# brucefan1983/GPUMD

Measured on AMD Instinct MI355X. Metric: atom-steps/sec, NEP PbTe NVE (nep4 2 Te Pb, examples/nep_train/nep.txt), higher is better.
Workload: dtype f32

## Files before the change

### gpumd_amd/csrc/capi_impl.h

```cpp
#pragma once
#include "../../include/nepmi.h"
#include "engine_impl.h"

#include <exception>
#include <string>

struct nepmi_api;
#if defined(NEPMI_CAPI_DISPATCH)
extern "C" const nepmi_api nepmi_self_api;
#define NEPMI_SELF_API (&nepmi_self_api)
#else
#define NEPMI_SELF_API nullptr
#endif

struct nepmi_model {
  const nepmi_api* api;
  nepmi::NepModel m;
};

struct nepmi_engine {
  const nepmi_api* api;
  nepmi::EngineT<NepmiBackend>* e;
};

// ... 584 lines not shown
  e->e->set_unwrapped(d_unwrapped);
  return NEPMI_OK;
}

int nepmi_engine_set_option(nepmi_engine* e, const char* name, double value)
{
  if (!e || !name)
    return fail(NEPMI_ERR_ARG, "null engine or option name");
  const std::string n(name);
  const int iv = (int)value;
  auto& eng = *e->e;
  if (n == "generic")
    return guarded([&] { eng.set_force_generic(iv != 0); });
  if (n == "tiles")
    eng.set_tile_mode(iv < 0 ? -1 : iv > 2 ? 2 : iv);
  else if (n == "win_lanes")
    eng.set_win_lanes(iv);
  else if (n == "win_max_atoms")
    eng.set_win_max_atoms(iv);
  else if (n == "scatter_guard")
    eng.set_scatter_guard_delayed(value, eng.take_guard_delay());
  else if (n == "scatter_guard_hard")
    eng.set_scatter_guard(-1.0, value);
  else if (n == "scatter_guard_delay")
    eng.set_guard_delay(iv);
  else if (n == "radial_mask")
    eng.set_radial_mask(iv != 0);
  else if (n == "radial_sync")
    eng.set_radial_sync(iv != 0);
  else if (n == "angular_fused")
    eng.set_angular_fused(iv != 0);
  else if (n == "angular_pair_trip")
    eng.set_angular_pair_trip(iv != 0);
  else if (n == "fold_seam")
    eng.set_fold_seam(iv != 0);
  else if (n == "brick_force") {
    if (iv != 0 && !eng.has_brick_force())
      return fail(NEPMI_ERR_ARG, "option 'brick_force': the per-brick force kernel is not part of this build (make BRICK=1)");
    eng.set_brick_force(iv != 0);
  }
  else if (n == "win_static")
    eng.set_win2(iv != 0);
  else if (n == "keep_lists_on_box_change")
    eng.set_keep_lists(iv != 0);
  else if (n == "stepwise_loops")
    eng.set_stepwise_loops(iv != 0);
  else if (n == "mfma")
    eng.set_use_mfma(iv);
  else if (n == "angular_recompute")
    eng.set_angular_recompute(iv);
  else
    return fail(NEPMI_ERR_ARG, "unknown engine option '" + n + "'");
  return NEPMI_OK;
}

}
```

### gpumd_amd/csrc/engine.hip

```cpp
#include <hip/hip_runtime.h>
#include <hiprand/hiprand_kernel.h>

#include <cstring>
#include <stdexcept>
#include <string>

#include "engine_impl.h"
#include "nep_scatter.h"
#include "nep_fused.h"
#ifndef NEPMI_WITH_BRICK
#define NEPMI_WITH_BRICK 0
#endif
#if NEPMI_WITH_BRICK
#include "experimental/nep_brick.h"
#endif

namespace nepmi {

#define NEPMI_HIP_CHECK(expr)                                                                       \
  do {                                                                                              \
    hipError_t err__ = (expr);                                                                      \
    if (err__ != hipSuccess)                                                                        \
      throw std::runtime_error(std::string("HIP error: ") + hipGetErrorString(err__) + " at " +     \
                               __FILE__ + ":" + std::to_string(__LINE__) + " (" #expr ")");         \
// ... 1386 lines not shown
    if (t)
      timer_start(timing->slot[slot]);
    hipLaunchKernelGGL((nepmi_kernel_lds_parts<BLOCK, P, Body>), dim3((unsigned)grid), dim3(BLOCK), lds_bytes, stream, body, n,
                       frozen);
    NEPMI_HIP_CHECK(hipGetLastError());
    if (t)
      timer_stop(timing->slot[slot]);
  }

  template <int BLOCK, class Body, bool SORTED = false>
  void launch_lds_pairs(int slot, int64_t n, const Body& body)
  {
    if (n <= 0)
      return;
    const int64_t grid = ((2 * n + BLOCK - 1) / BLOCK + 7) / 8 * 8;
    const size_t lds_bytes = ((size_t)body.lds_floats() * sizeof(float) + 15) / 16 * 16;
    void (*kern)(const Body, const int64_t, const int*) = nullptr;
    if constexpr (SORTED)
      kern = &nepmi_kernel_lds_pairs_sorted<BLOCK, Body>;
    else
      kern = &nepmi_kernel_lds_pairs<BLOCK, Body>;
    if (lds_bytes > 60 * 1024)
      NEPMI_HIP_CHECK(hipFuncSetAttribute(reinterpret_cast<const void*>(kern), hipFuncAttributeMaxDynamicSharedMemorySize, (int)lds_bytes));
    const bool t = timed(slot);
    if (t)
      timer_start(timing->slot[slot]);
    hipLaunchKernelGGL(kern, dim3((unsigned)grid), dim3(BLOCK), lds_bytes, stream, body, n, frozen);
    NEPMI_HIP_CHECK(hipGetLastError());
    if (t)
      timer_stop(timing->slot[slot]);
  }

  template <class S>
  size_t fused_image_floats(const ModelD& md) const
  {
    return (size_t)fused_lds_layout<S>(md).total;
  }
  template <class S>
  void launch_angular_fused(int slot, int64_t n, const ModelD& md, const Bufs& b, int export_qfp, float* img, bool build, bool pair_trip)
  {
    AngularFusedBody<S> body{md, b, export_qfp, nullptr};
    if (build) {
      hipLaunchKernelGGL((nepmi_fused_image<AngularFusedBody<S>>), dim3(1), dim3(256), 0, stream, body, img);
      NEPMI_HIP_CHECK(hipGetLastError());
    }
    body.img = img;
#ifndef NEPMI_AFU_BLOCK
#define NEPMI_AFU_BLOCK 256
#endif
#ifndef NEPMI_AFU_SORT
#define NEPMI_AFU_SORT 0
#endif
    if constexpr (FusedShape<S>::NLOC <= kFusedTripMaxChannels) {
      if (pair_trip) {
        launch_lds_pairs<NEPMI_AFU_BLOCK, AngularFusedBody<S, 1>, NEPMI_AFU_SORT != 0>(slot, n, AngularFusedBody<S, 1>{md, b, export_qfp, img});
        return;
      }
    }
    launch_lds_pairs<NEPMI_AFU_BLOCK, AngularFusedBody<S>, NEPMI_AFU_SORT != 0>(slot, n, body);
  }

  template <class S>
  size_t fused_window_lds_bytes(const ModelD& md) const
  {
    return (size_t)fused_lds_layout<S>(md, kFusedWindowTypes).total * sizeof(float);
  }
  static constexpr bool kHasFusedWindow = NEPMI_WITH_FUSED_WINDOW != 0;
  template <class S>
  void launch_angular_fused_window(int slot, int64_t n, const ModelD& md, const Bufs& b, int export_qfp, float* img, bool build)
  {
#if NEPMI_WITH_FUSED_WINDOW
    if (n <= 0)
      return;
    AngularFusedBody<S> body{md, b, export_qfp, nullptr};
    if (build) {
      hipLaunchKernelGGL((nepmi_fused_image<AngularFusedBody<S>>), dim3(1), dim3(256), 0, stream, body, img);
      NEPMI_HIP_CHECK(hipGetLastError());
    }
    body.img = img;
    body.tw = kFusedWindowTypes;
    const int64_t grid = ((n + 127) / 128 + 7) / 8 * 8;
    const size_t lds_bytes = (fused_window_lds_bytes<S>(md) + 15) / 16 * 16;
    if (lds_bytes > 64 * 1024)
      NEPMI_HIP_CHECK(hipFuncSetAttribute(reinterpret_cast<const void*>(&nepmi_fused_window_kernel<AngularFusedBody<S>>),
                                          hipFuncAttributeMaxDynamicSharedMemorySize, (int)lds_bytes));
    const bool t = timed(slot);
    if (t)
      timer_start(timing->slot[slot]);
    hipLaunchKernelGGL((nepmi_fused_window_kernel<AngularFusedBody<S>>), dim3((unsigned)grid), dim3(256), lds_bytes, stream, body, n, frozen);
    NEPMI_HIP_CHECK(hipGetLastError());
    if (t)
      timer_stop(timing->slot[slot]);
// ... 428 lines not shown
```

### gpumd_amd/csrc/engine_impl.h

```cpp
#pragma once
#include "nep_bodies.h"
#include "nep_md.h"
#include "nep_model.h"
#include "nep_window.h"
#include "nep_highl.h"
#include "tersoff_bodies.h"

#include <cmath>
#include <cstdio>
#include <cstring>
#include <string>
#include <random>
#include <vector>

#ifndef NEPMI_TERSOFF_SEAM
#define NEPMI_TERSOFF_SEAM 1
#endif
#ifndef NEPMI_WIN2_DEFAULT
#define NEPMI_WIN2_DEFAULT 1
#endif

#define NEPMI_UNPAREN(...) __VA_ARGS__
#if defined(NEPMI_JIT_CORE)
#define NEPMI_SHAPE_DISPATCH(FN, GENERIC, ARGS)                                   \
// ... 1569 lines not shown
                          T * T * ((model_.n_max_radial + 1) * (model_.basis_size_radial + 1) +
                                   (model_.n_max_angular + 1) * (model_.basis_size_angular + 1) + 1) + 8;
    return floats * sizeof(float) <= 64 * 1024;
  }
  bool ang_fused_window_active() const
  {
    if (!B::kHasFusedWindow || !B::kHasFusedAngular || !ang_fused_ || model_.kind != 0 || shape_ == 0 || ann_mode_ != 1 || model_.num_types <= 4 || !b_.fpr)
      return false;
    if ((model_.n_max_angular + 2) / 2 > 5)
      return false;
    const int nrh = (model_.n_max_radial + 2) / 2, nloc = (model_.n_max_angular + 2) / 2;
    const int dph = (nrh + model_.num_L * nloc + 3) / 4 * 4;
    const size_t T = (size_t)model_.num_types, tw = 4;
    const size_t floats = tw * ((size_t)model_.num_neurons * 2 * dph + 32 + 2 * model_.num_neurons) + 2 * dph +
                          tw * T * ((model_.n_max_angular + 1) * (model_.basis_size_angular + 1) + 1) + 16;
    return floats * sizeof(float) <= 80 * 1024;
  }
  template <class S>
  void launch_angular_fused_window(int export_qfp = 0)
  {
    if constexpr (B::kHasFusedWindow && B::kHasFusedAngular && S::fixed && S::TS == 0) {
      const size_t need = be_.template fused_image_floats<S>(md_);
      if (!fused_img_ || fused_img_floats_ < need) {
        dfree(fused_img_);
        fused_img_ = dalloc<float>(need);
        fused_img_floats_ = need;
        fused_img_stale_ = true;
      }
      be_.template launch_angular_fused_window<S>(kSlotAngular, N_, md_, b_, export_qfp, fused_img_, fused_img_stale_);
      fused_img_stale_ = false;
    }
  }
  template <class S>
  void launch_angular_fused(int export_qfp = 0)
  {
    if constexpr (B::kHasFusedAngular && S::fixed) {
      const size_t need = be_.template fused_image_floats<S>(md_);
      if (!fused_img_ || fused_img_floats_ < need) {
        dfree(fused_img_);
        fused_img_ = dalloc<float>(need);
        fused_img_floats_ = need;
        fused_img_stale_ = true;
      }
      be_.template launch_angular_fused<S>(kSlotAngular, N_, md_, b_, export_qfp, fused_img_, fused_img_stale_, ang_pair_trip_);
      fused_img_stale_ = false;
    }
  }

  template <class S>
  bool brick_force_wanted(const WinStage& ws2) const
  {
    if constexpr (!(B::kHasBrickForce && S::fixed && S::TS == 2)) {
      return false;
    } else {
      if (!brick_force_ || !ang_fused_active() || b_.level || b_.use_rmask || b_.use_csync || !scatter_wanted<S>(ws2))
        return false;
      return be_.template brick_lds_bytes<S>(md_, win_.wmax) <= B::kMaxLdsBytes;
    }
  }
  template <class S>
  void launch_brick_force(const WinStage& ws2, const int* frozen)
  {
    if constexpr (B::kHasBrickForce && S::fixed && S::TS == 2) {
      if (fused_img_stale_ || !fused_img_) {
        launch_angular_fused<S>(0);
      }
      be_.template launch_brick_force<S>(kSlotAngular, kSlotForce, num_bricks_, N_, ws2, md_, halo_, fmap_, fold_rows_, step_outputs_,
                                         fused_img_, frozen);
    }
  }

  template <class S>
  void launch_angular_force()
  {
    const bool big_table = (size_t)cang_floats(md_) * sizeof(float) > 16 * 1024;
#ifndef NEPMI_AF_PAIRS_BIG
#define NEPMI_AF_PAIRS_BIG 0
#endif
    if (S::fixed && S::NA + 1 >= 7)
      be_.template launch_lds_pairs<64>(kSlotAngForce, N_, AngularForceBody<S>{md_, b_, recompute_s()});
    else if (NEPMI_AF_PAIRS_BIG && S::fixed && big_table)
      be_.template launch_lds_pairs<512>(kSlotAngForce, N_, AngularForceBody<S>{md_, b_, recompute_s()});
    else if (big_table)
      be_.template launch_lds<512>(kSlotAngForce, N_, AngularForceBody<S>{md_, b_, recompute_s()});
    else
      be_.template launch_lds<64>(kSlotAngForce, N_, AngularForceBody<S>{md_, b_, recompute_s()});
    if (!S::fixed && model_.L_max > 4)
      be_.template launch<64>(kSlotAngForce, N_, HighLForceBody{md_, b_});
  }

#if defined(NEPMI_JIT_SHAPE)
  using S_JIT = Shape<NEPMI_JIT_SHAPE>;
#endif
  using S_PbTeA = Shape<6, 6, 6, 6, 5, 2>;
  using S_PbTeB = Shape<4, 8, 4, 8, 5, 2>;
  using S_C2022 = Shape<10, 10, 8, 8, 6, 1>;
  using S_UNEP = Shape<4, 8, 4, 8, 6, 0>;
  using S_BZO = Shape<8, 8, 6, 8, 5, 0>;
// ... 58 lines not shown
  }
  void set_external_skin(bool on) { external_skin_ = on; }
  void set_reverse_ghosts(bool on)
  {
    if (on && model_.kind != 0)
      throw EngineError{-4, "reverse-mode ghosts: NEP models only"};
    reverse_ghosts_ = on;
    b_.lvl_desc = on ? 2 : 1;
    b_.lvl_force = on ? 1 : 2;
    invalidate();
  }
  bool reverse_ghosts() const { return reverse_ghosts_; }
  void reset_thermostat() { nhc_fresh_ = true; }
  void set_unwrapped(double* u) { unwrapped_ = u; }
  void check_flags_now()
  {
    int flags[kNumFlags];
    be_.d2h(flags, b_.flags, sizeof(flags));
    check_overflow(flags);
  }
  void set_angular_recompute(int mode) { recompute_mode_ = mode; }
  void set_temperature(double temperature)
  {
    const NepModel& m = model_;
    if (!m.temperature_model || m.kind != 0 || temperature == temperature_)
      return;
    temperature_ = temperature;
    const float qT = (float)temperature * m.q_scaler_temp;
    b0_eff_.resize(m.b0.size());
    for (size_t k = 0; k < m.b0.size(); ++k)
      b0_eff_[k] = m.b0[k] - m.w0_temp[k] * qT;
    be_.h2d(const_cast<float*>(md_.b0), b0_eff_.data(), sizeof(float) * b0_eff_.size());
    be_.ann_prepare(md_, b_);
    fused_img_stale_ = true;
  }
  double temperature() const { return temperature_; }
  bool temperature_model() const { return model_.temperature_model; }
  int recompute_s() const
  {
    return recompute_mode_ < 0 ? (model_.MN_angular <= 16 ? 1 : 0) : (recompute_mode_ ? 1 : 0);
  }
  void adopt_from(const EngineT& o)
  {
    use_tiles_ = o.use_tiles_;
    tile_mode_ = o.tile_mode_;
    recompute_mode_ = o.recompute_mode_;
    win_lanes_ = o.win_lanes_;
    win_max_atoms_ = o.win_max_atoms_;
    use_win2_ = o.use_win2_;
    external_skin_ = o.external_skin_;
    force_form_ = o.force_form_;
    use_rmask_ = o.use_rmask_;
    use_csync_ = o.use_csync_;
    ang_fused_ = o.ang_fused_;
    ang_pair_trip_ = o.ang_pair_trip_;
    fold_seam_ = o.fold_seam_;
    brick_force_ = o.brick_force_;
    loop_ctx_ = o.loop_ctx_;
    scatter_disabled_ = o.scatter_disabled_;
    b_.scatter_limit = o.b_.scatter_limit;
    b_.fold_guard = o.b_.fold_guard;
    b_.scatter_hard = o.b_.scatter_hard;
    b_.fold_hard = o.b_.fold_hard;
    hard_factor_ = o.hard_factor_;
    hard_asked_ = o.hard_asked_;
    guard_delay_ = o.guard_delay_;
    guard_delayed_ = o.guard_delayed_;
    if (reverse_ghosts_ != o.reverse_ghosts_)
      set_reverse_ghosts(o.reverse_ghosts_);
    unwrapped_ = o.unwrapped_;
    nhc_fresh_ = o.nhc_fresh_;
    bdp_rng_ = o.bdp_rng_;
    bdp_iset_ = o.bdp_iset_;
    bdp_gset_ = o.bdp_gset_;
    lan_seed_ = o.lan_seed_;
    num_compute = o.num_compute;
    num_rebuild = o.num_rebuild;
    num_discarded = o.num_discarded;
    num_range_handovers = o.num_range_handovers;
    be_.adopt_options(o.be_);
    if (ann_mode_ != o.ann_mode_)
      set_use_mfma(o.ann_mode_);
    if (force_generic_ != o.force_generic_)
      set_force_generic(o.force_generic_);
    if (o.temperature_ != temperature_)
      set_temperature(o.temperature_);
    have_list_ = false;
  }
// ... 315 lines not shown
  void set_guard_delay(int n) { guard_delay_next_ = n > 0 ? n : 0; }
  int take_guard_delay()
  {
    const int n = guard_delay_next_;
    guard_delay_next_ = 0;
    return n;
  }
  void set_flagged_steps_stand(bool on)
  {
    b_.scatter_hard = on ? (float)(hard_factor_ * b_.scatter_limit) : 0.0f;
    b_.fold_hard = on ? (int)((hard_factor_ > 2.0 ? hard_factor_ : 2.0) * b_.scatter_limit * 4194304.0) : 0;
  }
  bool scatter_enabled() const { return !scatter_disabled_; }
  void clear_range_hard()
  {
    int ov = 0;
    be_.d2h(&ov, b_.flags + kFlagOverflow, sizeof(int));
    if (ov & kOverflowRangeHard) {
      ov &= ~kOverflowRangeHard;
      be_.h2d(b_.flags + kFlagOverflow, &ov, sizeof(int));
    }
  }
  void disable_scatter()
  {
    if (!scatter_disabled_)
      ++num_range_handovers;
    scatter_disabled_ = true;
    be_.memset(b_.flags + kFlagRange, 0, sizeof(int));
  }
  bool last_scatter_form() const { return last_scatter_form_; }
  void set_angular_fused(bool on) { ang_fused_ = on; }
  void set_angular_pair_trip(bool on) { ang_pair_trip_ = on; }
  bool ang_pair_trip_active() const { return ang_pair_trip_ && (model_.n_max_angular + 2) / 2 <= 4; }
  void set_fold_seam(bool on) { fold_seam_ = on; }
  void set_brick_force(bool on) { brick_force_ = on; }
  static constexpr bool has_brick_force() { return B::kHasBrickForce; }
  void set_loop_context(bool on) { loop_ctx_ = on; }
  void set_step_outputs(bool on) { step_outputs_ = on; }
  bool loop_context() const { return loop_ctx_; }
  void exact_virials()
  {
    if (!virial_local_ || model_.kind != 0 || last_small_)
      return;
    be_.frozen = nullptr;
    NEPMI_SHAPE_DISPATCH(exact_virials_shape, 1, ())
  }
  bool virial_local() const { return virial_local_; }

private:
  template <class S>
  void compact_lists_shape()
  {
    const bool padded_rows = b_.use_csync != 0;
    force_kernels_shape<S>(kPhaseRadialOnly, nullptr);
    if (padded_rows)
      angular_kernels<S>();
  }
  template <class S>
  void exact_virials_shape()
  {
    const WinStage ws{box_, b_, win_};
    WinLayout lay2 = win_;
    lay2.compact = 1;
    const WinStage ws2{box_, b_, lay2};
    const int lanes = win_lanes();
    if (!ccode_valid_)
// ... 50 lines not shown
  std::string describe() const
  {
    static const char* shapes[] = {"generic", "PbTe-A(6,6,6,6,5;2)", "PbTe-B(4,8,4,8,5;2)", "C-2022(10,10,8,8,6;1)", "UNEP(4,8,4,8,6;T)",
                                   "BaZrO3(8,8,6,8,5;T)"};
    std::string s;
    if (model_.kind == 1)
      return "potential=tersoff1989 kernels=bond_order+force(fp64)";
    if (shape_ == 6) {
      char jb[96];
      std::snprintf(jb, sizeof jb, "shape=jit(%d,%d,%d,%d,%d;%s)", model_.n_max_radial, model_.basis_size_radial, model_.n_max_angular,
                    model_.basis_size_angular, model_.num_L, model_.num_types <= 2 ? std::to_string(model_.num_types).c_str() : "T");
      s += jb;
    } else {
      if (shape_ == 7 || shape_ == 8 || shape_ == 9) {
        s += shape_ == 7 ? "shape=cover(8,12,8,12,6;T)" : (shape_ == 8 ? "shape=cover(12,16,10,12,6;T)" : "shape=cover(8,12,8,12,6;2)");
        if (model_.embedded()) {
          char eb[128];
          std::snprintf(eb, sizeof eb, "<-zero_padded_model(%d,%d,%d,%d,%d)", model_.file_n_max_radial, model_.file_basis_size_radial,
                        model_.file_n_max_angular, model_.file_basis_size_angular, model_.file_num_L);
          s += eb;
        }
      } else {
        s += std::string("shape=") + shapes[shape_ >= 0 && shape_ <= 5 ? shape_ : 0];
      }
    }
    if (last_small_)
      return s + " path=small_box(all image pairs)";
    const int lanes = win_lanes();
    const bool win2 = win2_ok_ && lanes == 1;
    s += tile_ok_ ? (win2 ? " window=lds_static" : " window=lds_scanned") : " window=none(gather kernels)";
    s += " lanes_per_atom=" + std::to_string(tile_ok_ ? lanes : 1);
    if (last_brick_)
      s += " force=one_kernel_per_brick(descriptor+ann+partial_forces+lds_scatter_of_own_halves,lane_pairs)";
    else if (last_ang_fused_)
      s += last_ang_window_ ? " angular=descriptor+ann+partial_forces_in_one_kernel(lane_pairs,sums_in_registers,type_sorted,window_of_4_types)"
                            : (ang_pair_trip_active() ? " angular=descriptor+ann+partial_forces_in_one_kernel(lane_pairs,sums_in_registers,two_record_trips)"
                                              : " angular=descriptor+ann+partial_forces_in_one_kernel(lane_pairs,sums_in_registers)");
    else if (fuse_ann_active())
      s += " ann=fused_with_angular_descriptor(packed_fp32,no_mfma)";
    else if (ann_mode_ != 0 && b_.ann_img && (model_.num_types <= 4 || b_.skip_atab))
      s += model_.num_types > 4 ? " ann=mfma_f32_32x32x2(one_type_per_workgroup)" : " ann=mfma_f32_32x32x2";
    else
      s += " ann=per_atom";
    if (!last_ang_fused_) {
      s += (shape_ != 0 && model_.n_max_angular + 1 >= 7) ? " angular_force=lane_pairs" : " angular_force=one_lane";
      s += recompute_s() ? " angular_sums=recomputed" : " angular_sums=stored";
    }
    s += (last_scatter_form_ && last_mask_form_)   ? " radial_list=inside_bits_over_the_verlet_words"
         : (last_scatter_form_ && last_sync_form_) ? " radial_list=wave_synchronous_words"
                                                   : " radial_list=compacted";
    s += last_scatter_form_ ? (last_fold_seam_ ? " force_assembly=lds_scatter_of_own_halves(fixed_point)+fold_in_integrator_pass"
                                               : " force_assembly=lds_scatter_of_own_halves(fixed_point)+fold") :
         last_rows_form_ ? " force_assembly=table_rows_in_lds"
                         : (last_fpj_form_ ? " force_assembly=neighbour_half_from_fp_rows" : " force_assembly=table_rows_gathered");
    if (num_seam_vetoes_ > 0)
      s += " seam_vetoes=" + std::to_string(num_seam_vetoes_);
    if (tile_ok_)
      s += " bricks=" + std::to_string(num_bricks_) + " window_slots=" + std::to_string(win_.wmax);
    return s;
  }
  void force_kernels(int phase, const int* frozen = nullptr)
  {
    be_.frozen = frozen;
    force_kernels_dispatch(phase, frozen);
    be_.frozen = nullptr;
    step_outputs_ = true;
    assembly_part_ = 0;
  }
  void force_kernels_on(B& side, int phase, const int* frozen)
  {
// ... 12 lines not shown
    if (model_.kind == 1) {
      be_.begin_region(kRegionForce);
      if (N_ < 200000)
        be_.template launch_lds_parts<kTersoffBlock, kTersoffLanes>(kSlotRadial, N_, TersoffPartialBody{box_, tp_, b_, tb_, kTersoffLanes});
      else
        be_.template launch_lds<kTersoffBlock>(kSlotRadial, N_, TersoffPartialBody{box_, tp_, b_, tb_});
      if (tersoff_defer_)
        tersoff_deferred_ = true;
      else
        be_.template launch<64>(kSlotForce, N_, TersoffAssembleBody{b_, tb_});
      be_.end_region(kRegionForce);
      return;
    }
    NEPMI_SHAPE_DISPATCH(force_kernels_shape, 1, (phase, frozen))
  }

  NepModel model_;
  B be_;
  int64_t cap_;
  int64_t N_;
  ModelD md_{};
  Bufs b_;
  BoxD box_;
  WinLayout win_{0, 0};
  bool win2_ok_ = false, use_win2_ = NEPMI_WIN2_DEFAULT != 0;
  bool use_rows_ = true;
  bool last_rows_form_ = false, last_fpj_form_ = false, last_scatter_form_ = false;
  int force_form_ = -1;
  bool loop_ctx_ = false;
  bool virial_local_ = false;
  double hard_factor_ = 4.0;
  bool ang_fused_ = true;
  bool ang_pair_trip_ = !(std::getenv("NEPMI_ANGULAR_PAIR_TRIP") && std::atoi(std::getenv("NEPMI_ANGULAR_PAIR_TRIP")) == 0);
  bool brick_force_ = false;
  bool last_brick_ = false;
  bool brick_pending_ = false;
  float* fused_img_ = nullptr;
  size_t fused_img_floats_ = 0;
  bool fused_img_stale_ = true;
  bool last_ang_fused_ = false;
  bool use_rmask_ = false;
  bool last_mask_form_ = false;
  bool last_ang_window_ = false;
  bool last_sync_form_ = false;
  int guard_delay_ = 0;
  int guard_delay_next_ = 0;
  bool fold_seam_ = !(std::getenv("NEPMI_FOLD_SEAM") && std::atoi(std::getenv("NEPMI_FOLD_SEAM")) == 0);
  bool fold_defer_ = false;
  bool fold_deferred_ = false;
  static constexpr int kSeamBackoffSteps = 256;
  int seam_backoff_ = 0;
  int64_t num_seam_vetoes_ = 0;
  bool last_fold_seam_ = false;
  bool tersoff_defer_ = false;
  bool tersoff_deferred_ = false;
  int64_t calm_steps_ = 0;
  int* brick_live_buf_ = nullptr;
  double* thermo_rows_ = nullptr;
  int64_t thermo_rows_cap_ = 0;
  bool rev_valid_ = false;
  const int* dmap_dev_ = nullptr;
  double hard_asked_ = 4.0;
  double guard_delayed_ = 64.0;
  bool use_csync_ = true;
  bool ccode_valid_ = true;
  bool step_outputs_ = true;
// ... 73 lines not shown
```

### gpumd_amd/csrc/nep_fused.h

```cpp
#pragma once
#include "nep_window.h"

namespace nepmi {

template <class S>
struct FusedShape {
  static_assert(S::fixed, "compiled shapes only");
  static constexpr int NRH = (S::NR + 2) / 2;
  static constexpr int NLOC = (S::NA + 2) / 2;
  static constexpr int DPH = (NRH + S::NL * NLOC + 3) / 4 * 4;
  NEPMI_HD static int component(int part, int i)
  {
    if (i < NRH) {
      const int n = 2 * i + part;
      return n <= S::NR ? n : -1;
    }
    const int ii = i - NRH, L = ii / NLOC, c = ii - L * NLOC, n = 2 * c + part;
    if (L >= S::NL || n > S::NA)
      return -1;
    return (S::NR + 1) + L * (S::NA + 1) + n;
  }
};

constexpr int kFusedTripMaxChannels = 4;

struct FusedLdsLayout {
  int wstride, off_w, off_b0, off_w1, off_c, off_qs, total;
};
template <class S>
NEPMI_HD FusedLdsLayout fused_lds_layout(const ModelD& m, int TW = 0)
{
  using F = FusedShape<S>;
  const int tw = TW > 0 ? TW : m.T;
  FusedLdsLayout a;
  a.wstride = m.nneu * 2 * F::DPH;
  a.wstride += (8 - (a.wstride & 31) + 32) & 31;
  a.off_w = (tw * m.T * cang_stride(m) + 3) / 4 * 4;
  a.off_b0 = a.off_w + tw * a.wstride;
  a.off_w1 = a.off_b0 + tw * m.nneu;
  a.off_c = a.off_w1 + tw * m.nneu;
  a.off_qs = a.off_c + (TW > 0 ? 0 : m.T * m.T * (m.NR + 1) * (m.KR + 1));
  a.off_qs = (a.off_qs + 3) / 4 * 4;
  a.total = (a.off_qs + 2 * F::DPH + 3) / 4 * 4;
  return a;
}

template <class S, int TRIP = 0>
struct AngularFusedBody {
  ModelD m;
  Bufs b;
  int export_qfp;
  const float* img;
  int tw = 0;
  static constexpr bool kUsesLds = true;
#ifndef NEPMI_AFU_WAVES
#define NEPMI_AFU_WAVES 2
#endif
#ifndef NEPMI_AFU_ABL
#define NEPMI_AFU_ABL 0
#endif
#ifndef NEPMI_AFU_NJ
#define NEPMI_AFU_NJ 1
#endif
  static constexpr int kMinWavesPerEu = 1, kMinWavesPerEuPairs = NEPMI_AFU_WAVES;
  using F = FusedShape<S>;

  NEPMI_HD int lds_floats() const { return fused_lds_layout<S>(m, tw).total; }
  NEPMI_HD void stage_window(float* dst, int tb, int nt, int tid, int nth) const
  {
    const FusedLdsLayout G = fused_lds_layout<S>(m, 0), A = fused_lds_layout<S>(m, tw);
    const int cs = cang_stride(m);
    {
      const float* src = img + (size_t)tb * m.T * cs;
      for (int i = tid; i < nt * m.T * cs; i += nth)
        dst[i] = src[i];
    }
    {
      const F4f* __restrict__ src = reinterpret_cast<const F4f*>(img + G.off_w + (size_t)tb * G.wstride);
      F4f* d4 = reinterpret_cast<F4f*>(dst + A.off_w);
      for (int i = tid; i < nt * A.wstride / 4; i += nth)
        d4[i] = src[i];
    }
    for (int i = tid; i < nt * m.nneu; i += nth) {
      dst[A.off_b0 + i] = img[G.off_b0 + tb * m.nneu + i];
      dst[A.off_w1 + i] = img[G.off_w1 + tb * m.nneu + i];
    }
    for (int i = tid; i < 2 * F::DPH; i += nth)
      dst[A.off_qs + i] = img[G.off_qs + i];
  }
  NEPMI_HD void lds_stage(float* dst, int tid, int nth) const
  {
    if (img) {
      const int n4 = (fused_lds_layout<S>(m).total + 3) / 4;
      const F4f* __restrict__ src = reinterpret_cast<const F4f*>(img);
      F4f* d4 = reinterpret_cast<F4f*>(dst);
      for (int i = tid; i < n4; i += nth)
        d4[i] = src[i];
      return;
    }
    cang_stage(m, dst, tid, nth);
    const FusedLdsLayout a = fused_lds_layout<S>(m);
    const int per_t = m.nneu * 2 * F::DPH;
    for (int idx = tid; idx < m.T * per_t; idx += nth) {
      const int t = idx / per_t, r = idx - t * per_t;
      const int j = r / (2 * F::DPH), pi = r - j * (2 * F::DPH);
      const int p = pi / F::DPH, i = pi - p * F::DPH;
      const int d = F::component(p, i);
      dst[a.off_w + t * a.wstride + r] = d >= 0 ? m.w0[((size_t)t * m.nneu + j) * m.dim + d] : 0.0f;
    }
    for (int idx = tid; idx < m.T * m.nneu; idx += nth) {
      dst[a.off_b0 + idx] = m.b0[idx];
      dst[a.off_w1 + idx] = m.w1[idx];
    }
    for (int idx = tid; idx < m.T * m.T * (m.NR + 1) * (m.KR + 1); idx += nth)
      dst[a.off_c + idx] = m.c_rad[idx];
    for (int idx = tid; idx < 2 * F::DPH; idx += nth) {
      const int d = F::component(idx / F::DPH, idx % F::DPH);
      dst[a.off_qs + idx] = d >= 0 ? m.qscale[d] : 0.0f;
    }
  }

  NEPMI_HD int sort_key(int64_t k) const
  {
    if (b.lvl[k] < b.lvl_desc)
      return 0;
    return (b.use_csync && b.nn_angtrue) ? b.nn_angtrue[k] : b.nn_angstep[k];
  }
  template <int PARTS, class LP>
  NEPMI_HD void run_parts(int64_t k, int part, LP lds) const
  {
    static_assert(PARTS == 2, "lane pairs");
    run_window(k, part, lds, 0);
  }
  template <class LP>
  NEPMI_HD void run_window(int64_t k, int part, LP lds, int tb) const
  {
    constexpr int NLOC = F::NLOC, DPH = F::DPH;
    if (b.lvl[k] < b.lvl_desc)
      return;
    const int t1 = b.posq[k].type;
    LP cang = lds - tb * m.T * cang_stride(m);
    float s[NLOC * kNumHarm], Fp[DPH], e;
    descriptor_and_ann(k, part, lds, cang, t1, t1 - tb, s, Fp, e);
    if (part == 0)
      b.pe_i[k] = e;
    if (b.fpr) {
#pragma unroll
      for (int i = 0; i < F::NRH; ++i) {
        const int n = 2 * i + part;
        if (n <= S::NR)
          b.fpr[(size_t)k * b.FPR + n] = Fp[i];
      }
    }
    if (!b.skip_atab && tw == 0 && NEPMI_AFU_ABL != 4) {
      constexpr int KRPC = (S::KR + 1 + 3) / 4 * 4;
      const int KRP = b.KRP;
      for (int t2 = 0; t2 < m.T; ++t2) {
        float row[KRPC];
        radial_row(part, lds, t1, t2, Fp, row);
        if ((t2 & 1) == part) {
          F4f* __restrict__ out = reinterpret_cast<F4f*>(b.atab + (size_t)k * (m.T * KRP) + t2 * KRP);
#pragma unroll
          for (int g = 0; g < KRPC / 4; ++g)
            out[g] = F4f{row[4 * g], row[4 * g + 1], row[4 * g + 2], row[4 * g + 3]};
        }
      }
    }
    if (b.level && !b.angf[k])
      return;
    adjoint_in_place(part, Fp, s);
    const AngularForceBody<S> af{m, b, 1};
    if (NEPMI_AFU_ABL != 2) {
      if constexpr (TRIP)
        af.pairs_from_G_trip(k, part, cang, t1, s, typename AngularForceBody<S>::F12Store{b.f12 + k, b.N});
      else
        af.template pairs_from_G<2>(k, part, cang, t1, s, typename AngularForceBody<S>::F12Store{b.f12 + k, b.N});
    } else if (s[3] + s[NLOC * kNumHarm - 1] == 12345.0f) {
      b.pe_i[k] = s[5] + s[NLOC * kNumHarm - 2];
    }
  }

  template <class LP>
  NEPMI_HD void radial_row(int part, LP lds, int t1, int t2, const float* Fp, float* row) const
  {
    constexpr int NRH = F::NRH;
    constexpr int KRPC = (S::KR + 1 + 3) / 4 * 4;
    const FusedLdsLayout a = fused_lds_layout<S>(m);
    LP c = lds + a.off_c + (t1 * m.T + t2) * (S::NR + 1) * (S::KR + 1);
#pragma unroll
    for (int kk = 0; kk < KRPC; ++kk) {
      float v = 0.0f;
      if (kk <= S::KR) {
#pragma unroll
        for (int i = 0; i < NRH; ++i) {
          const int n = 2 * i + part;
          if (n <= S::NR)
            v = fmaf(Fp[i], c[n * (S::KR + 1) + kk], v);
        }
        v += NEPMI_PAIR_XCHG(v);
      }
      row[kk] = v;
    }
  }

  NEPMI_HD void adjoint_in_place(int part, const float* Fp, float* s) const
  {
    constexpr int NRH = F::NRH, NLOC = F::NLOC;
#pragma unroll
    for (int i = 0; i < NLOC; ++i) {
      const int n = part + 2 * i;
      if (n > S::NA)
        break;
      float fpn[S::kRows];
#pragma unroll
      for (int L = 0; L < S::kRows; ++L)
        fpn[L] = L < S::NL ? Fp[NRH + (L < S::NL ? L : 0) * NLOC + i] : 0.0f;
      invariants_adjoint<false>(m, fpn, 1, &s[i * kNumHarm]);
    }
  }

  template <class LP>
  NEPMI_HD void descriptor_and_ann(int64_t k, int part, LP lds, LP cang, int t1, int tl, float* s, float* Fp, float& e_out) const
  {
    constexpr int NRH = F::NRH, NLOC = F::NLOC, DPH = F::DPH;
    const int64_t N = b.N;
    const FusedLdsLayout a = fused_lds_layout<S>(m, tw);
    const int64_t gk = b.tpos[k];
    LP QS = lds + a.off_qs + part * DPH;

    if (NEPMI_AFU_ABL != 3) {
      if constexpr (TRIP)
        angular_s_sums_trip<S>(m, b, k, t1, cang, part, s);
      else
        angular_s_sums<S, 2>(m, b, k, t1, cang, part, s);
    } else {
#pragma unroll
      for (int i = 0; i < NLOC * kNumHarm; ++i)
        s[i] = (float)(k & 15) * 0.01f + 0.001f * i;
    }

    float ql[DPH];
#pragma unroll
    for (int i = 0; i < DPH; ++i)
      ql[i] = 0.0f;
#pragma unroll
    for (int i = 0; i < NRH; ++i) {
      const int n = 2 * i + part;
      if (n <= S::NR)
        ql[i] = b.q[(int64_t)n * N + gk];
    }
#pragma unroll
    for (int i = 0; i < NLOC; ++i) {
      const int n = part + 2 * i;
      if (n > S::NA)
        break;
      float qn[S::kRows];
#pragma unroll
      for (int L = 0; L < S::kRows; ++L)
        qn[L] = 0.0f;
      invariants<false>(m, &s[i * kNumHarm], qn, 1);
#pragma unroll
      for (int L = 0; L < S::NL; ++L) {
        ql[NRH + L * NLOC + i] = qn[L] * QS[NRH + L * NLOC + i];
        if (export_qfp)
          b.q[(int64_t)((S::NR + 1) + L * (S::NA + 1) + n) * N + gk] = ql[NRH + L * NLOC + i];
      }
    }

    f2 g2[DPH / 2];
#pragma unroll
    for (int i = 0; i < DPH / 2; ++i)
      g2[i] = bc2(0.0f);
    float e = 0.0f;
    {
      LP W = lds + a.off_w + tl * a.wstride + part * DPH;
      LP B0 = lds + a.off_b0 + tl * m.nneu;
      LP W1 = lds + a.off_w1 + tl * m.nneu;
      constexpr bool kKeepRow = DPH <= 24;
      constexpr int NJ = kKeepRow ? NEPMI_AFU_NJ : 1;
      auto neurons = [&](const int j0, const int nj) __attribute__((always_inline)) {
        f2 w2[NJ][kKeepRow ? DPH / 2 : 1];
        f2 acc0[NJ], acc1[NJ];
#pragma unroll
        for (int u = 0; u < NJ; ++u) {
          if (u >= nj)
            break;
          LP w = W + (j0 + u) * (2 * DPH);
          acc0[u] = bc2(0.0f);
          acc1[u] = bc2(0.0f);
#pragma unroll
          for (int i = 0; i < DPH / 2; ++i) {
            const f2 wv = mk2(w[2 * i], w[2 * i + 1]);
            if (kKeepRow)
              w2[u][i] = wv;
            if (i & 1)
              acc1[u] = vfma(wv, mk2(ql[2 * i], ql[2 * i + 1]), acc1[u]);
            else
              acc0[u] = vfma(wv, mk2(ql[2 * i], ql[2 * i + 1]), acc0[u]);
          }
        }
#pragma unroll
        for (int u = 0; u < NJ; ++u) {
          if (u >= nj)
            break;
          LP w = W + (j0 + u) * (2 * DPH);
          const f2 acc = acc0[u] + acc1[u];
          float dot = acc.x + acc.y;
          dot += NEPMI_PAIR_XCHG(dot);
          const float h = ann_tanh(dot - B0[j0 + u]);
          const float wj = W1[j0 + u];
          e = fmaf(wj, h, e);
          const f2 coef = bc2(wj * (1.0f - h * h));
#pragma unroll
          for (int i = 0; i < DPH / 2; ++i)
            g2[i] = vfma(coef, kKeepRow ? w2[u][i] : mk2(w[2 * i], w[2 * i + 1]), g2[i]);
        }
      };
      int j = 0;
      for (; j + NJ <= (NEPMI_AFU_ABL == 1 ? 0 : m.nneu); j += NJ)
        neurons(j, NJ);
      if (NJ > 1 && j < m.nneu)
        neurons(j, m.nneu - j);
    }
    e_out = e - (m.b1 + m.b1t[t1]);
#pragma unroll
    for (int i = 0; i < DPH; ++i)
      Fp[i] = ((i & 1) ? g2[i >> 1].y : g2[i >> 1].x) * QS[i];
    if (export_qfp) {
#pragma unroll
      for (int i = 0; i < DPH; ++i) {
        const int d = F::component(part, i);
        if (d >= 0)
          b.fp[(int64_t)d * N + gk] = Fp[i];
      }
    }
  }
};

}
```

### gpumd_amd/nep.py

```python
import ctypes as C

import numpy as np

from . import _capi


def _h9(box):
    h = np.ascontiguousarray(np.asarray(box, dtype=np.float64).reshape(9))
    return h, h.ctypes.data_as(_capi.c_dp)


def _pbc3(pbc):
    p = np.ascontiguousarray(np.asarray(pbc, dtype=np.int32).reshape(3))
    return p, p.ctypes.data_as(_capi.c_ip)


class Model:

    def __init__(self, path, lib=None):
        from . import load_library
        self.lib = lib if lib is not None else load_library()
        self.path = path
        self.handle = self.lib.nepmi_model_load(path.encode())
        if not self.handle:
# ... 279 lines not shown

    def set_tiles(self, mode=-1):
        mode = 2 if mode is True else 0 if mode is False else int(mode)
        self.set_option("tiles", mode)

    def set_win_lanes(self, lanes=0):
        self.set_option("win_lanes", int(lanes))

    def set_force_form(self, mode=-1):
        self._ck(self.lib.nepmi_engine_set_force_form(self.handle, int(mode)))

    def set_radial_mask(self, on=True):
        self.set_option("radial_mask", 1 if on else 0)

    def set_radial_sync(self, on=True):
        self.set_option("radial_sync", 1 if on else 0)

    def set_scatter_guard(self, ev_per_angstrom=64.0, hard_factor=0.0):
        self.set_option("scatter_guard", float(ev_per_angstrom))
        self.set_option("scatter_guard_hard", float(hard_factor))

    def set_virial_mode(self, mode=0):
        self._ck(self.lib.nepmi_engine_set_virial_mode(self.handle, int(mode)))

    def set_brick_force(self, on=True):
        self.set_option("brick_force", 1 if on else 0)

    def set_angular_fused(self, on=True):
        self.set_option("angular_fused", 1 if on else 0)

    def set_angular_pair_trip(self, on=True):
        self.set_option("angular_pair_trip", 1 if on else 0)

    def set_fold_seam(self, on=True):
        self.set_option("fold_seam", 1 if on else 0)

    def describe(self):
        import ctypes as C
        buf = C.create_string_buffer(512)
        n = self.lib.nepmi_engine_describe(self.handle, buf, 512)
        if n < 0:
            self._ck(n)
        return buf.value.decode()

    def set_stepwise_loops(self, on=True):
        self.set_option("stepwise_loops", int(bool(on)))

    def set_win_static(self, on=True):
        self.set_option("win_static", int(bool(on)))

    def set_mfma(self, on=True):
        self.set_option("mfma", int(on))

    def set_temperature(self, temperature):
        self._ck(self.lib.nepmi_engine_set_temperature(self.handle, float(temperature)))

    def set_angular_recompute(self, mode=-1):
        self.set_option("angular_recompute", int(mode))

    def set_generic(self, on=True):
        self.set_option("generic", 1 if on else 0)
```

Before: 954.0 million.

## Add flat LDS table layout for fused angular kernel, enabled by default

Adds a 'flat' variant of the fused angular kernel's LDS image. It interleaves b0 and w1 per neuron and repacks the radial coefficient table per (t1,t2,part), padding the k dimension to a multiple of four so the radial-row projection can read contiguous blocks. The new radial_rows_flat path loads coefficients for two neighbour types at once into registers. Descriptor scalers are also held in registers, and the early-exit check is hoisted in the pair-trip variant. It is on by default and adds a separate image buffer and more kernel template instantiations, with more register pressure from the wider coefficient arrays.

```diff
diff --git a/gpumd_amd/csrc/capi_impl.h b/gpumd_amd/csrc/capi_impl.h
--- a/gpumd_amd/csrc/capi_impl.h
+++ b/gpumd_amd/csrc/capi_impl.h
@@ -640,6 +640,8 @@
     eng.set_angular_fused(iv != 0);
   else if (n == "angular_pair_trip")
     eng.set_angular_pair_trip(iv != 0);
+  else if (n == "angular_flat_tables")
+    eng.set_angular_flat_tables(iv != 0);
   else if (n == "fold_seam")
     eng.set_fold_seam(iv != 0);
   else if (n == "brick_force") {
diff --git a/gpumd_amd/csrc/engine.hip b/gpumd_amd/csrc/engine.hip
--- a/gpumd_amd/csrc/engine.hip
+++ b/gpumd_amd/csrc/engine.hip
@@ -1442,32 +1442,47 @@
   }
 
   template <class S>
-  size_t fused_image_floats(const ModelD& md) const
-  {
-    return (size_t)fused_lds_layout<S>(md).total;
+  size_t fused_image_floats(const ModelD& md, bool flat = false) const
+  {
+    return (size_t)fused_lds_layout<S>(md, 0, flat ? 1 : 0).total;
   }
   template <class S>
-  void launch_angular_fused(int slot, int64_t n, const ModelD& md, const Bufs& b, int export_qfp, float* img, bool build, bool pair_trip)
-  {
-    AngularFusedBody<S> body{md, b, export_qfp, nullptr};
+  void launch_angular_fused(int slot, int64_t n, const ModelD& md, const Bufs& b, int export_qfp, float* img, bool build, bool pair_trip,
+                            bool flat = false)
+  {
     if (build) {
-      hipLaunchKernelGGL((nepmi_fused_image<AngularFusedBody<S>>), dim3(1), dim3(256), 0, stream, body, img);
+      if (flat)
+        hipLaunchKernelGGL((nepmi_fused_image<AngularFusedBody<S, 0, 1>>), dim3(1), dim3(256), 0, stream,
+                           AngularFusedBody<S, 0, 1>{md, b, export_qfp, nullptr}, img);
+      else
+        hipLaunchKernelGGL((nepmi_fused_image<AngularFusedBody<S>>), dim3(1), dim3(256), 0, stream,
+                           AngularFusedBody<S>{md, b, export_qfp, nullptr}, img);
       NEPMI_HIP_CHECK(hipGetLastError());
     }
-    body.img = img;
 #ifndef NEPMI_AFU_BLOCK
 #define NEPMI_AFU_BLOCK 256
 #endif
 #ifndef NEPMI_AFU_SORT
 #define NEPMI_AFU_SORT 0
 #endif
-    if constexpr (FusedShape<S>::NLOC <= kFusedTripMaxChannels) {
+    constexpr bool kTrips = FusedShape<S>::NLOC <= kFusedTripMaxChannels;
+    if (flat) {
+      if constexpr (kTrips) {
+        if (pair_trip) {
+          launch_lds_pairs<NEPMI_AFU_BLOCK, AngularFusedBody<S, 1, 1>, NEPMI_AFU_SORT != 0>(slot, n, AngularFusedBody<S, 1, 1>{md, b, export_qfp, img});
+          return;
+        }
+      }
+      launch_lds_pairs<NEPMI_AFU_BLOCK, AngularFusedBody<S, 0, 1>, NEPMI_AFU_SORT != 0>(slot, n, AngularFusedBody<S, 0, 1>{md, b, export_qfp, img});
+      return;
+    }
+    if constexpr (kTrips) {
       if (pair_trip) {
         launch_lds_pairs<NEPMI_AFU_BLOCK, AngularFusedBody<S, 1>, NEPMI_AFU_SORT != 0>(slot, n, AngularFusedBody<S, 1>{md, b, export_qfp, img});
         return;
       }
     }
-    launch_lds_pairs<NEPMI_AFU_BLOCK, AngularFusedBody<S>, NEPMI_AFU_SORT != 0>(slot, n, body);
+    launch_lds_pairs<NEPMI_AFU_BLOCK, AngularFusedBody<S>, NEPMI_AFU_SORT != 0>(slot, n, AngularFusedBody<S>{md, b, export_qfp, img});
   }
 
   template <class S>
diff --git a/gpumd_amd/csrc/engine_impl.h b/gpumd_amd/csrc/engine_impl.h
--- a/gpumd_amd/csrc/engine_impl.h
+++ b/gpumd_amd/csrc/engine_impl.h
@@ -1625,9 +1625,22 @@
     }
   }
   template <class S>
-  void launch_angular_fused(int export_qfp = 0)
+  void launch_angular_fused(int export_qfp = 0, bool classic_image = false)
   {
     if constexpr (B::kHasFusedAngular && S::fixed) {
+      if (ang_flat_tables_ && !classic_image) {
+        const size_t need = be_.template fused_image_floats<S>(md_, true);
+        if (!fused_img_flat_ || fused_img_flat_floats_ < need) {
+          dfree(fused_img_flat_);
+          fused_img_flat_ = dalloc<float>(need);
+          fused_img_flat_floats_ = need;
+          fused_img_flat_stale_ = true;
+        }
+        be_.template launch_angular_fused<S>(kSlotAngular, N_, md_, b_, export_qfp, fused_img_flat_, fused_img_flat_stale_, ang_pair_trip_, true);
+        fused_img_flat_stale_ = false;
+        last_ang_flat_ = true;
+        return;
+      }
       const size_t need = be_.template fused_image_floats<S>(md_);
       if (!fused_img_ || fused_img_floats_ < need) {
         dfree(fused_img_);
@@ -1637,6 +1650,7 @@
       }
       be_.template launch_angular_fused<S>(kSlotAngular, N_, md_, b_, export_qfp, fused_img_, fused_img_stale_, ang_pair_trip_);
       fused_img_stale_ = false;
+      last_ang_flat_ = false;
     }
   }
 
@@ -1656,7 +1670,7 @@
   {
     if constexpr (B::kHasBrickForce && S::fixed && S::TS == 2) {
       if (fused_img_stale_ || !fused_img_) {
-        launch_angular_fused<S>(0);
+        launch_angular_fused<S>(0, true);
       }
       be_.template launch_brick_force<S>(kSlotAngular, kSlotForce, num_bricks_, N_, ws2, md_, halo_, fmap_, fold_rows_, step_outputs_,
                                          fused_img_, frozen);
@@ -1781,7 +1795,7 @@
       b0_eff_[k] = m.b0[k] - m.w0_temp[k] * qT;
     be_.h2d(const_cast<float*>(md_.b0), b0_eff_.data(), sizeof(float) * b0_eff_.size());
     be_.ann_prepare(md_, b_);
-    fused_img_stale_ = true;
+    fused_img_stale_ = fused_img_flat_stale_ = true;
   }
   double temperature() const { return temperature_; }
   bool temperature_model() const { return model_.temperature_model; }
@@ -1803,6 +1817,7 @@
     use_csync_ = o.use_csync_;
     ang_fused_ = o.ang_fused_;
     ang_pair_trip_ = o.ang_pair_trip_;
+    ang_flat_tables_ = o.ang_flat_tables_;
     fold_seam_ = o.fold_seam_;
     brick_force_ = o.brick_force_;
     loop_ctx_ = o.loop_ctx_;
@@ -2184,6 +2199,7 @@
   void set_angular_fused(bool on) { ang_fused_ = on; }
   void set_angular_pair_trip(bool on) { ang_pair_trip_ = on; }
   bool ang_pair_trip_active() const { return ang_pair_trip_ && (model_.n_max_angular + 2) / 2 <= 4; }
+  void set_angular_flat_tables(bool on) { ang_flat_tables_ = on; }
   void set_fold_seam(bool on) { fold_seam_ = on; }
   void set_brick_force(bool on) { brick_force_ = on; }
   static constexpr bool has_brick_force() { return B::kHasBrickForce; }
@@ -2300,10 +2316,11 @@
     s += " lanes_per_atom=" + std::to_string(tile_ok_ ? lanes : 1);
     if (last_brick_)
       s += " force=one_kernel_per_brick(descriptor+ann+partial_forces+lds_scatter_of_own_halves,lane_pairs)";
+    else if (last_ang_fused_ && last_ang_window_)
+      s += " angular=descriptor+ann+partial_forces_in_one_kernel(lane_pairs,sums_in_registers,type_sorted,window_of_4_types)";
     else if (last_ang_fused_)
-      s += last_ang_window_ ? " angular=descriptor+ann+partial_forces_in_one_kernel(lane_pairs,sums_in_registers,type_sorted,window_of_4_types)"
-                            : (ang_pair_trip_active() ? " angular=descriptor+ann+partial_forces_in_one_kernel(lane_pairs,sums_in_registers,two_record_trips)"
-                                              : " angular=descriptor+ann+partial_forces_in_one_kernel(lane_pairs,sums_in_registers)");
+      s += std::string(" angular=descriptor+ann+partial_forces_in_one_kernel(lane_pairs,sums_in_registers") +
+           (ang_pair_trip_active() ? ",two_record_trips" : "") + (last_ang_flat_ ? ",flat_tables)" : ")");
     else if (fuse_ann_active())
       s += " ann=fused_with_angular_descriptor(packed_fp32,no_mfma)";
     else if (ann_mode_ != 0 && b_.ann_img && (model_.num_types <= 4 || b_.skip_atab))
@@ -2382,6 +2399,11 @@
   double hard_factor_ = 4.0;
   bool ang_fused_ = true;
   bool ang_pair_trip_ = !(std::getenv("NEPMI_ANGULAR_PAIR_TRIP") && std::atoi(std::getenv("NEPMI_ANGULAR_PAIR_TRIP")) == 0);
+  bool ang_flat_tables_ = !(std::getenv("NEPMI_ANGULAR_FLAT_TABLES") && std::atoi(std::getenv("NEPMI_ANGULAR_FLAT_TABLES")) == 0);
+  float* fused_img_flat_ = nullptr;
+  size_t fused_img_flat_floats_ = 0;
+  bool fused_img_flat_stale_ = true;
+  bool last_ang_flat_ = false;
   bool brick_force_ = false;
   bool last_brick_ = false;
   bool brick_pending_ = false;
diff --git a/gpumd_amd/csrc/nep_fused.h b/gpumd_amd/csrc/nep_fused.h
--- a/gpumd_amd/csrc/nep_fused.h
+++ b/gpumd_amd/csrc/nep_fused.h
@@ -28,7 +28,7 @@
   int wstride, off_w, off_b0, off_w1, off_c, off_qs, total;
 };
 template <class S>
-NEPMI_HD FusedLdsLayout fused_lds_layout(const ModelD& m, int TW = 0)
+NEPMI_HD FusedLdsLayout fused_lds_layout(const ModelD& m, int TW = 0, int flat = 0)
 {
   using F = FusedShape<S>;
   const int tw = TW > 0 ? TW : m.T;
@@ -37,6 +37,14 @@
   a.wstride += (8 - (a.wstride & 31) + 32) & 31;
   a.off_w = (tw * m.T * cang_stride(m) + 3) / 4 * 4;
   a.off_b0 = a.off_w + tw * a.wstride;
+  if (flat && TW == 0) {
+    constexpr int KRPC = (S::KR + 1 + 3) / 4 * 4;
+    a.off_w1 = a.off_b0 + 1;
+    a.off_c = (a.off_b0 + 2 * tw * m.nneu + 3) / 4 * 4;
+    a.off_qs = a.off_c + m.T * m.T * 2 * F::NRH * KRPC;
+    a.total = (a.off_qs + 2 * F::DPH + 3) / 4 * 4;
+    return a;
+  }
   a.off_w1 = a.off_b0 + tw * m.nneu;
   a.off_c = a.off_w1 + tw * m.nneu;
   a.off_qs = a.off_c + (TW > 0 ? 0 : m.T * m.T * (m.NR + 1) * (m.KR + 1));
@@ -45,7 +53,7 @@
   return a;
 }
 
-template <class S, int TRIP = 0>
+template <class S, int TRIP = 0, int FLAT = 0>
 struct AngularFusedBody {
   ModelD m;
   Bufs b;
@@ -64,8 +72,10 @@
 #endif
   static constexpr int kMinWavesPerEu = 1, kMinWavesPerEuPairs = NEPMI_AFU_WAVES;
   using F = FusedShape<S>;
-
-  NEPMI_HD int lds_floats() const { return fused_lds_layout<S>(m, tw).total; }
+  static constexpr bool kRoomy = F::NLOC <= kFusedTripMaxChannels;
+
+  NEPMI_HD FusedLdsLayout layout() const { return fused_lds_layout<S>(m, tw, FLAT); }
+  NEPMI_HD int lds_floats() const { return layout().total; }
   NEPMI_HD void stage_window(float* dst, int tb, int nt, int tid, int nth) const
   {
     const FusedLdsLayout G = fused_lds_layout<S>(m, 0), A = fused_lds_layout<S>(m, tw);
@@ -91,7 +101,7 @@
   NEPMI_HD void lds_stage(float* dst, int tid, int nth) const
   {
     if (img) {
-      const int n4 = (fused_lds_layout<S>(m).total + 3) / 4;
+      const int n4 = (fused_lds_layout<S>(m, 0, FLAT).total + 3) / 4;
       const F4f* __restrict__ src = reinterpret_cast<const F4f*>(img);
       F4f* d4 = reinterpret_cast<F4f*>(dst);
       for (int i = tid; i < n4; i += nth)
@@ -99,7 +109,7 @@
       return;
     }
     cang_stage(m, dst, tid, nth);
-    const FusedLdsLayout a = fused_lds_layout<S>(m);
+    const FusedLdsLayout a = fused_lds_layout<S>(m, 0, FLAT);
     const int per_t = m.nneu * 2 * F::DPH;
     for (int idx = tid; idx < m.T * per_t; idx += nth) {
       const int t = idx / per_t, r = idx - t * per_t;
@@ -108,12 +118,27 @@
       const int d = F::component(p, i);
       dst[a.off_w + t * a.wstride + r] = d >= 0 ? m.w0[((size_t)t * m.nneu + j) * m.dim + d] : 0.0f;
     }
-    for (int idx = tid; idx < m.T * m.nneu; idx += nth) {
-      dst[a.off_b0 + idx] = m.b0[idx];
-      dst[a.off_w1 + idx] = m.w1[idx];
-    }
-    for (int idx = tid; idx < m.T * m.T * (m.NR + 1) * (m.KR + 1); idx += nth)
-      dst[a.off_c + idx] = m.c_rad[idx];
+    if constexpr (FLAT) {
+      constexpr int KRPC = (S::KR + 1 + 3) / 4 * 4, BLK = 2 * F::NRH * KRPC;
+      for (int idx = tid; idx < m.T * m.nneu; idx += nth) {
+        dst[a.off_b0 + 2 * idx] = m.b0[idx];
+        dst[a.off_b0 + 2 * idx + 1] = m.w1[idx];
+      }
+      for (int idx = a.off_b0 + 2 * m.T * m.nneu + tid; idx < a.off_c; idx += nth)
+        dst[idx] = 0.0f;
+      for (int idx = tid; idx < m.T * m.T * BLK; idx += nth) {
+        const int blk = idx / BLK, r = idx - blk * BLK;
+        const int p = r / (F::NRH * KRPC), i = (r / KRPC) % F::NRH, kk = r % KRPC, n = 2 * i + p;
+        dst[a.off_c + idx] = (n <= S::NR && kk <= S::KR) ? m.c_rad[(blk * (S::NR + 1) + n) * (S::KR + 1) + kk] : 0.0f;
+      }
+    } else {
+      for (int idx = tid; idx < m.T * m.nneu; idx += nth) {
+        dst[a.off_b0 + idx] = m.b0[idx];
+        dst[a.off_w1 + idx] = m.w1[idx];
+      }
+      for (int idx = tid; idx < m.T * m.T * (m.NR + 1) * (m.KR + 1); idx += nth)
+        dst[a.off_c + idx] = m.c_rad[idx];
+    }
     for (int idx = tid; idx < 2 * F::DPH; idx += nth) {
       const int d = F::component(idx / F::DPH, idx % F::DPH);
       dst[a.off_qs + idx] = d >= 0 ? m.qscale[d] : 0.0f;
@@ -136,8 +161,13 @@
   NEPMI_HD void run_window(int64_t k, int part, LP lds, int tb) const
   {
     constexpr int NLOC = F::NLOC, DPH = F::DPH;
-    if (b.lvl[k] < b.lvl_desc)
+    if constexpr (FLAT && TRIP) {
+      const int lv = b.lvl[k], ty = b.posq[k].type, sl = b.tpos[k], na = b.nn_angstep[k];
+      if ((lv < b.lvl_desc) | ((ty | sl | na) < 0))
+        return;
+    } else if (b.lvl[k] < b.lvl_desc) {
       return;
+    }
     const int t1 = b.posq[k].type;
     LP cang = lds - tb * m.T * cang_stride(m);
     float s[NLOC * kNumHarm], Fp[DPH], e;
@@ -152,7 +182,9 @@
           b.fpr[(size_t)k * b.FPR + n] = Fp[i];
       }
     }
-    if (!b.skip_atab && tw == 0 && NEPMI_AFU_ABL != 4) {
+    if (FLAT && !b.skip_atab && tw == 0 && NEPMI_AFU_ABL != 4) {
+      radial_rows_flat(k, part, lds, t1, Fp);
+    } else if (!b.skip_atab && tw == 0 && NEPMI_AFU_ABL != 4) {
       constexpr int KRPC = (S::KR + 1 + 3) / 4 * 4;
       const int KRP = b.KRP;
       for (int t2 = 0; t2 < m.T; ++t2) {
@@ -203,6 +235,77 @@
     }
   }
 
+  template <class LP>
+  NEPMI_HD void radial_rows_flat(int64_t k, int part, LP lds, int t1, const float* Fp) const
+  {
+    constexpr int NRH = F::NRH;
+    constexpr int KRPC = (S::KR + 1 + 3) / 4 * 4;
+    const FusedLdsLayout a = layout();
+    const int KRP = b.KRP;
+    if constexpr (!kRoomy) {
+      for (int t2 = 0; t2 < m.T; ++t2) {
+        LP p = lds + a.off_c + ((t1 * m.T + t2) * 2 + part) * (NRH * KRPC);
+        F4f* __restrict__ out = reinterpret_cast<F4f*>(b.atab + (size_t)k * (m.T * KRP) + t2 * KRP);
+#pragma unroll
+        for (int g = 0; g < KRPC / 4; ++g) {
+          float c[NRH][4], v[4];
+#pragma unroll
+          for (int i = 0; i < NRH; ++i)
+#pragma unroll
+            for (int j = 0; j < 4; ++j)
+              c[i][j] = p[i * KRPC + 4 * g + j];
+#pragma unroll
+          for (int j = 0; j < 4; ++j) {
+            v[j] = 0.0f;
+            if (4 * g + j <= S::KR) {
+#pragma unroll
+              for (int i = 0; i < NRH; ++i)
+                v[j] = fmaf(Fp[i], c[i][j], v[j]);
+              v[j] += NEPMI_PAIR_XCHG(v[j]);
+            }
+          }
+          if ((t2 & 1) == part)
+            out[g] = F4f{v[0], v[1], v[2], v[3]};
+        }
+      }
+      return;
+    }
+    for (int t2 = 0; t2 < m.T; t2 += 2) {
+      const int t2b = t2 + 1 < m.T ? t2 + 1 : t2;
+      float c[2][NRH][KRPC];
+#pragma unroll
+      for (int u = 0; u < 2; ++u) {
+        LP p = lds + a.off_c + ((t1 * m.T + (u ? t2b : t2)) * 2 + part) * (NRH * KRPC);
+#pragma unroll
+        for (int i = 0; i < NRH; ++i)
+#pragma unroll
+          for (int kk = 0; kk < KRPC; ++kk)
+            c[u][i][kk] = p[i * KRPC + kk];
+      }
+#pragma unroll
+      for (int u = 0; u < 2; ++u) {
+        float row[KRPC];
+#pragma unroll
+        for (int kk = 0; kk < KRPC; ++kk) {
+          float v = 0.0f;
+          if (kk <= S::KR) {
+#pragma unroll
+            for (int i = 0; i < NRH; ++i)
+              v = fmaf(Fp[i], c[u][i][kk], v);
+            v += NEPMI_PAIR_XCHG(v);
+          }
+          row[kk] = v;
+        }
+        if (u == part && t2 + u < m.T) {
+          F4f* __restrict__ out = reinterpret_cast<F4f*>(b.atab + (size_t)k * (m.T * KRP) + (t2 + u) * KRP);
+#pragma unroll
+          for (int g = 0; g < KRPC / 4; ++g)
+            out[g] = F4f{row[4 * g], row[4 * g + 1], row[4 * g + 2], row[4 * g + 3]};
+        }
+      }
+    }
+  }
+
   NEPMI_HD void adjoint_in_place(int part, const float* Fp, float* s) const
   {
     constexpr int NRH = F::NRH, NLOC = F::NLOC;
@@ -224,7 +327,7 @@
   {
     constexpr int NRH = F::NRH, NLOC = F::NLOC, DPH = F::DPH;
     const int64_t N = b.N;
-    const FusedLdsLayout a = fused_lds_layout<S>(m, tw);
+    const FusedLdsLayout a = layout();
     const int64_t gk = b.tpos[k];
     LP QS = lds + a.off_qs + part * DPH;
 
@@ -249,6 +352,13 @@
       if (n <= S::NR)
         ql[i] = b.q[(int64_t)n * N + gk];
     }
+    constexpr bool kScalersInRegisters = FLAT && kRoomy;
+    float qs[kScalersInRegisters ? DPH : 1];
+    if constexpr (kScalersInRegisters) {
+#pragma unroll
+      for (int i = 0; i < DPH; ++i)
+        qs[i] = QS[i];
+    }
 #pragma unroll
     for (int i = 0; i < NLOC; ++i) {
       const int n = part + 2 * i;
@@ -261,8 +371,23 @@
       invariants<false>(m, &s[i * kNumHarm], qn, 1);
 #pragma unroll
       for (int L = 0; L < S::NL; ++L) {
-        ql[NRH + L * NLOC + i] = qn[L] * QS[NRH + L * NLOC + i];
-        if (export_qfp)
+        if constexpr (kScalersInRegisters) {
+          ql[NRH + L * NLOC + i] = qn[L] * qs[NRH + L * NLOC + i];
+        } else {
+          ql[NRH + L * NLOC + i] = qn[L] * QS[NRH + L * NLOC + i];
+          if (export_qfp)
+            b.q[(int64_t)((S::NR + 1) + L * (S::NA + 1) + n) * N + gk] = ql[NRH + L * NLOC + i];
+        }
+      }
+    }
+    if (kScalersInRegisters && export_qfp) {
+#pragma unroll
+      for (int i = 0; i < NLOC; ++i) {
+        const int n = part + 2 * i;
+        if (n > S::NA)
+          break;
+#pragma unroll
+        for (int L = 0; L < S::NL; ++L)
           b.q[(int64_t)((S::NR + 1) + L * (S::NA + 1) + n) * N + gk] = ql[NRH + L * NLOC + i];
       }
     }
@@ -274,8 +399,9 @@
     float e = 0.0f;
     {
       LP W = lds + a.off_w + tl * a.wstride + part * DPH;
-      LP B0 = lds + a.off_b0 + tl * m.nneu;
-      LP W1 = lds + a.off_w1 + tl * m.nneu;
+      constexpr int BWS = FLAT ? 2 : 1;
+      LP B0 = lds + a.off_b0 + tl * (BWS * m.nneu);
+      LP W1 = FLAT ? B0 + 1 : lds + a.off_w1 + tl * m.nneu;
       constexpr bool kKeepRow = DPH <= 24;
       constexpr int NJ = kKeepRow ? NEPMI_AFU_NJ : 1;
       auto neurons = [&](const int j0, const int nj) __attribute__((always_inline)) {
@@ -307,8 +433,8 @@
           const f2 acc = acc0[u] + acc1[u];
           float dot = acc.x + acc.y;
           dot += NEPMI_PAIR_XCHG(dot);
-          const float h = ann_tanh(dot - B0[j0 + u]);
-          const float wj = W1[j0 + u];
+          const float h = ann_tanh(dot - B0[BWS * (j0 + u)]);
+          const float wj = W1[BWS * (j0 + u)];
           e = fmaf(wj, h, e);
           const f2 coef = bc2(wj * (1.0f - h * h));
 #pragma unroll
diff --git a/gpumd_amd/nep.py b/gpumd_amd/nep.py
--- a/gpumd_amd/nep.py
+++ b/gpumd_amd/nep.py
@@ -335,6 +335,9 @@
     def set_angular_pair_trip(self, on=True):
         self.set_option("angular_pair_trip", 1 if on else 0)
 
+    def set_angular_flat_tables(self, on=True):
+        self.set_option("angular_flat_tables", 1 if on else 0)
+
     def set_fold_seam(self, on=True):
         self.set_option("fold_seam", 1 if on else 0)
 
```

Result: faster. 968.7 million (median of 6 runs) (+1.5%).
